# SYNCC-IN/hyperscanning-signal-analysis

Hardware: AMD Instinct MI355X
Metric: MVAR+ffDTF windows/sec, 2x32-ch dyad p=8, 256 freqs (higher is better)
Workload: dtype f64; 1 GPU; C2: 1 dyad(s)/GPU, 2x32 ch @500 Hz, 10 min, 2 s windows 50% overlap (599 windows per dyad), MVAR p=8, 256 freqs 0.5-128 Hz; dyads_per_gpu=1, k1=hop blocks summed once, shared by the overlapping windows (hop 500), k2=block Levinson-Whittle recursion, one workgroup per window, one launch, normalisation=inside K3 (rows of window w by workgroups of window w+lag), parallelism=dyad-sharded x1, gather=none

## Files before the change

hyperscanning_signal_analysis_amd/_lib.py:

```python
from __future__ import annotations

import ctypes
import os
from ctypes import POINTER, c_char_p, c_double, c_int, c_int32, c_int64, c_void_p

_HERE = os.path.dirname(os.path.abspath(__file__))
LIB_PATH = os.path.join(_HERE, "libhypermvar.so")

SIGNATURES = {
    "hmv_version": (c_int, []),
    "hmv_last_error": (c_char_p, []),
    "hmv_pad": (c_int, [c_int]),
    "hmv_set_tuning": (c_int, [c_int, c_int64]),
    "hmv_get_tuning": (c_int64, [c_int]),
    "hmv_yw_workspace_doubles": (c_int64, [c_int, c_int]),
    "hmv_lagcov_f64": (c_int, [c_void_p, c_int64, c_int64, c_void_p, c_void_p, c_int64, c_int, c_int, c_int,
                               c_void_p, c_void_p]),
    "hmv_lagcov_regular_workspace_doubles": (c_int64, [c_int64, c_int, c_int, c_int64, c_int]),
    "hmv_lagcov_regular_f64": (c_int, [c_void_p, c_int64, c_int64, c_int64, c_int64, c_int64, c_int, c_int, c_int,
                                       c_void_p, c_void_p, c_void_p]),
    "hmv_yw_solve_f64": (c_int, [c_void_p, c_int64, c_int, c_int, c_void_p, c_void_p, c_void_p, c_void_p,
                                 c_void_p, c_int64, c_void_p]),
    "hmv_twiddles_f64": (c_int, [c_void_p, c_int, c_double, c_int, c_void_p, c_void_p]),
    "hmv_tf_workspace_doubles": (c_int64, [c_int64, c_int, c_int]),
# ... 95 lines not shown
    "hmv_residuals_workspace_bytes": (c_int64, [c_int64, c_int, c_int]),
    "hmv_residuals_f64": (c_int, [c_void_p, c_int64, c_int64, c_void_p, c_void_p, c_int64, c_int, c_int, c_int, c_void_p,
                                  c_void_p, c_int64, c_void_p, c_int64, c_void_p]),
    "hmv_whiteness_f64": (c_int, [c_void_p, c_int64, c_int, c_int, c_int, c_double] + [c_void_p] * 6),
    "hmv_model_validation_workspace_bytes": (c_int64, [c_int64, c_int, c_int, c_int, c_int]),
    "hmv_model_validation_f64": (c_int, [c_void_p, c_int64, c_int64, c_void_p, c_void_p, c_int64, c_int, c_int, c_int,
                                         c_void_p, c_int, c_double] + [c_void_p] * 7 + [c_int64, c_void_p, c_int64, c_int64,
                                                                                       c_void_p]),
}

FLAG_UNFUSED_NORM = 1
FLAG_YW_TILED = 2
FLAG_YW_ONE_LAUNCH = 4
FLAG_DIRECT_LAGCOV = 8
MEASURE_FFDTF = 0
MEASURE_DDTF = 1
MEASURE_GPDC = 2
CRITERIA = {"AIC": 0, "HQ": 1, "SC": 2}
TUNE_NORM_LAG = 1
TUNE_LAG_GROUP = 2
TUNE_K3_FORM = 3
TUNE_YW_FORM = 4
TUNE_K3_LDS_PAD = 5


_lib = None


class HypermvarLibraryError(ImportError):
    pass


def load():
    global _lib
    if _lib is not None:
        return _lib
    global LIB_PATH
    LIB_PATH = os.environ.get("HYPERMVAR_LIB", LIB_PATH)
    if not os.path.exists(LIB_PATH):
        raise HypermvarLibraryError(
            f"{LIB_PATH} not found: build the HIP library first "
            f"(python -c 'import __graft_entry__ as g; g.build()' or make -C {_HERE}/csrc). "
            "There is no CPU fallback for the MVAR/ffDTF path.")
    lib = ctypes.CDLL(LIB_PATH)
    for name, (res, args) in SIGNATURES.items():
        try:
# ... 17 lines not shown
```

hyperscanning_signal_analysis_amd/csrc/capi.hip:

```cpp
#include "../../include/hypermvar.h"
#include "hmv_kernels.h"

#include <atomic>
#include <cmath>
#include <cstdio>
#include <cstdlib>
#include <cstring>

namespace {
thread_local char g_err[256] = "";

int fail(int code, const char* msg) {
  snprintf(g_err, sizeof(g_err), "%s", msg);
  return code;
}
int pad_of(int m) { return (m < 1 || m > HMV_MAX_CHANNELS) ? -1 : ((m + 15) / 16) * 16; }
inline hipStream_t S(void* s) { return reinterpret_cast<hipStream_t>(s); }
inline size_t align256(size_t b) { return (b + 255) & ~size_t(255); }

constexpr int N_TUNE = 6;
struct TuneRange { long long lo, hi; };
constexpr TuneRange kTuneRange[N_TUNE] = {{0, 0}, {0, 1 << 20}, {0, 3}, {0, 2}, {0, 4}, {0, 140000}};
long long env_knob(const char* name, int key) {
  const char* e = getenv(name);
  if (!e || !*e) return 0;
  char* end = nullptr;
  const long long v = strtoll(e, &end, 10);
  if (end == e || *end != 0 || v < kTuneRange[key].lo || v > kTuneRange[key].hi) {
    fprintf(stderr, "hypermvar: ignoring %s=%s (not an integer in %lld..%lld)\n", name, e, kTuneRange[key].lo,
            kTuneRange[key].hi);
    return 0;
  }
  return v;
}
std::atomic<long long> g_tune[N_TUNE] = {{0}, {env_knob("HYPERMVAR_NORM_LAG", 1)}, {env_knob("HYPERMVAR_LAG_GROUP", 2)},
                                         {env_knob("HYPERMVAR_K3_FORM", 3)}, {env_knob("HYPERMVAR_YW_FORM", 4)},
                                         {env_knob("HYPERMVAR_K3_LDS_PAD", 5)}};
}

namespace hmv {
long long tuning(int key) { return (key >= 1 && key < N_TUNE) ? g_tune[key].load(std::memory_order_relaxed) : -1; }
}

#ifdef HMV_STAMP
static unsigned long long* g_tf_stamps = nullptr;
extern "C" void hmv_debug_set_tf_stamps(void* p) { g_tf_stamps = static_cast<unsigned long long*>(p); }
#endif

extern "C" {

int hmv_version(void) { return HMV_VERSION; }
const char* hmv_last_error(void) { return g_err; }
int hmv_pad(int m) { return pad_of(m); }

int hmv_set_tuning(int key, int64_t value) {
  if (key < 1 || key >= N_TUNE) return fail(-1, "hmv_set_tuning: unknown key");
  if (value < kTuneRange[key].lo || value > kTuneRange[key].hi) return fail(-1, "hmv_set_tuning: value out of range");
  g_tune[key].store(value, std::memory_order_relaxed);
  return 0;
}
// ... 403 lines not shown
    o += align256(sizeof(double) * (size_t)(n < lag ? n : lag) * F * t);
  }
  w.total = o;
  return w;
}
int64_t norm_lag_items(int mp, int F) {
  const int64_t slots = (mp == 64 || mp == 48) ? 1024 : (mp == 32 ? 2048 : 5120);
  int64_t lag = (6 * slots + F - 1) / (F < 1 ? 1 : F);
  if (const int64_t t = hmv::tuning(HMV_TUNE_NORM_LAG)) lag = t;
  return lag < 8 ? 8 : lag;
}
}

int64_t hmv_tf_ffdtf_workspace_bytes(int64_t n_items, int m, int p, int F) {
  const int mp = pad_of(m);
  if (mp < 0 || n_items < 0 || p < 1 || F < 1) return -1;
  return (int64_t)tf_ff_layout(n_items, mp, p, F).total;
}

namespace {
int tf_ffdtf_impl(const char* who, const double* ar, int64_t n_items, int m, int p, const double* tw, int F, double* ffdtf,
                  double* band_out, const int32_t* bin_lo, const int32_t* bin_hi, int n_bands, double* den, double* H,
                  int32_t* info, double pivot_tau, void* workspace, int64_t workspace_bytes, int64_t flags,
                  void* ev_k3_start, void* ev_k3_stop, void* stream, const double* yw_ws = nullptr) {
  auto failw = [&](int code, const char* msg) {
    char buf[200];
    snprintf(buf, sizeof(buf), "%s: %s", who, msg);
    return fail(code, buf);
  };
  const int mp = pad_of(m);
  const bool bands = (band_out != nullptr);
  if (mp < 0) return failw(-1, "channel count must be in 1..64");
  if (p < 1) return failw(-2, "model order must be >= 1");
  if (n_items == 0) return 0;
  if (!ar || !tw || (!ffdtf && !bands) || !den || !info || !workspace || n_items < 0 || F < 1)
    return failw(-4, "null pointer / empty grid");
  if (!(pivot_tau > 0.0) || pivot_tau > 1.0) return failw(-6, "pivot_tau must be in (0, 1]");
  if (bands) {
    if (!bin_lo || !bin_hi || n_bands < 1) return failw(-4, "band bins missing");
    if (F % 32 != 0 || F > hmv::tf_band_max_F(mp) || (flags & HMV_FLAG_UNFUSED_NORM))
      return failw(-10, "in-kernel band sums need F % 32 == 0, F within the row worker's LDS block and the fused normalisation");
  }
  const TfFfWs w = tf_ff_layout(n_items, mp, p, F, bands);
  if ((int64_t)w.total > workspace_bytes) return failw(-7, "workspace too small");
  char* base = static_cast<char*>(workspace);
  const size_t t = (size_t)mp * mp;
  hmv::TfArgs a{};
  a.ar = ar; a.arx = reinterpret_cast<double*>(base + w.off_arx); a.tw = tw;
  a.P = reinterpret_cast<double*>(base + w.off_P); a.rowsum = reinterpret_cast<double*>(base + w.off_rowsum);
  a.H = H;
  a.info = info; a.n_items = n_items; a.F = F; a.p = p; a.m = m; a.tau = pivot_tau;
  const bool fused = bands || (!(flags & HMV_FLAG_UNFUSED_NORM) && (F % 16 == 0) && (reinterpret_cast<uintptr_t>(ffdtf) % 16 == 0));
  const int64_t lag = norm_lag_items(mp, F);
  const int64_t n_fused = fused ? n_items : 0;
  if (n_fused > 0) {
    a.ff = bands ? nullptr : ffdtf; a.den = den; a.fuse_items = n_fused; a.lag = (int)lag;
    if (bands) {
      a.bands = band_out; a.band_lo = reinterpret_cast<const int*>(bin_lo); a.band_hi = reinterpret_cast<const int*>(bin_hi);
      a.nb = n_bands;
    }
    a.wcount = reinterpret_cast<int*>(base + w.off_cnt);
    a.ready = a.wcount + n_items;
    a.missed = a.ready + n_items;
  }
#ifdef HMV_STAMP
  a.stamps = g_tf_stamps;
#endif
  hipStream_t st = S(stream);
  int rc = hmv::launch_tf_inv(a, mp, st, reinterpret_cast<hipEvent_t>(ev_k3_start), reinterpret_cast<hipEvent_t>(ev_k3_stop),
                              yw_ws);
  if (rc) return rc;
  if (n_fused < n_items) {
    const int64_t n_tail = n_items - n_fused;
    double* tail = bands ? reinterpret_cast<double*>(base + w.off_tail) : ffdtf + (size_t)n_fused * m * m * F;
    rc = hmv_ffdtf_norm_f64(a.P + (size_t)n_fused * F * t, a.rowsum + (size_t)n_fused * F * mp, den + (size_t)n_fused * mp,
                            tail, n_tail, F, m, 1, stream);
    if (!rc && bands)
      rc = hmv::launch_band_sums(tail, reinterpret_cast<const int*>(bin_lo), reinterpret_cast<const int*>(bin_hi),
                                 band_out + (size_t)n_fused * m * m * n_bands, n_tail * (long long)m * m, F, n_bands, st);
  }
  return rc;
}
}

int64_t hmv_tf_ffdtf_bands_workspace_bytes(int64_t n_items, int m, int p, int F) {
  const int mp = pad_of(m);
  if (mp < 0 || n_items < 0 || p < 1 || F < 1) return -1;
  return (int64_t)tf_ff_layout(n_items, mp, p, F, true).total;
}

int hmv_tf_ffdtf_f64(const double* ar, int64_t n_items, int m, int p, const double* tw, int F, double* ffdtf,
                     double* den, double* H, int32_t* info, double pivot_tau, void* workspace, int64_t workspace_bytes,
                     int64_t flags, void* ev_k3_start, void* ev_k3_stop, void* stream) {
// ... 42 lines not shown
}
int64_t sliding_bytes(int64_t chunk, int m, int p, int F, int n_bands = 0, bool spectra = false, int measure = MEAS_FFDTF,
                      int64_t q_tiles = -1) {
  const int mp = pad_of(m);
  if (mp < 0 || chunk < 1 || p < 1 || p > HMV_MAX_ORDER || F < 1 || n_bands < 0 || measure < MEAS_FFDTF ||
      measure > MEAS_GPDC)
    return -1;
  return (int64_t)sliding_layout(chunk, mp, p, F, n_bands > 0, spectra, measure, q_tiles).total;
}
struct ForkJoin {
  hipEvent_t fork = nullptr, join = nullptr;
};
ForkJoin* fork_join_events() {
  constexpr int MAXDEV = 64;
  thread_local ForkJoin tl[MAXDEV];
  int dev = 0;
  if (hipGetDevice(&dev) != hipSuccess || dev < 0 || dev >= MAXDEV) return nullptr;
  ForkJoin& e = tl[dev];
  if (!e.fork) {
    if (hipEventCreateWithFlags(&e.fork, hipEventDisableTiming) != hipSuccess) return nullptr;
    if (hipEventCreateWithFlags(&e.join, hipEventDisableTiming) != hipSuccess) return nullptr;
  }
  return &e;
}
}

int64_t hmv_sliding_workspace_bytes(int64_t chunk, int m, int p, int F) { return sliding_bytes(chunk, m, p, F); }

namespace {
struct EnsDesc {
  const int64_t* trial_rec;
  const int64_t* trial_start;
  const int64_t* group_ptr;
  int64_t n_groups, T;
  const int64_t* trial_rec_b = nullptr;
  const int64_t* trial_start_b = nullptr;
  int split = 0;
  const double* R_base = nullptr;
  const int64_t* item_base = nullptr;
};
struct PairDesc {
  const int64_t* rec_b;
  int split;
  const double* R_base;
  const int64_t* base_a;
  const int64_t* base_b;
// ... 70 lines not shown
  if (bands && (!a.bin_lo || !a.bin_hi || a.n_bands < 1)) return fail(-4, "hmv_sliding_ffdtf_f64: band bins missing");
  bool ens_shared = false;
  if (a.ens) {
    if (!a.ens->trial_rec || !a.ens->trial_start || !a.ens->group_ptr)
      return fail(-4, "hmv_sliding_ffdtf_f64: null pointer / empty grid");
    if (a.ens->n_groups < 1) return fail(-10, "hmv_sliding_ffdtf_f64: n_groups must be >= 1");
    if (a.grid_hop != 0 && !ens_grid_ok(a.n_items, a.ens->n_groups, a.n, a.ld, a.ens->T, a.grid_hop, a.grid_nwin))
      return fail(-9, "hmv_sliding_ffdtf_f64: inconsistent regular window grid");
    ens_shared = !a.ens->split && ens_shared_form(a.n, a.p, a.grid_hop, a.flags);
  }
  const SlidingWs w = sliding_layout(a.chunk, mp, a.p, a.F, bands, a.S_out != nullptr, a.measure,
                                     a.ens ? (ens_shared ? ens_q_tiles(a.chunk, a.n, a.p, a.grid_hop, a.grid_nwin) : 0)
                                           : ((a.pairs || a.mix) ? 0 : -1));
  if ((int64_t)w.total > a.workspace_bytes) return fail(-7, "hmv_sliding_ffdtf_f64: workspace too small");
  bool regular = !a.ens && !a.pairs && !a.mix && a.grid_hop > 0 && !(a.flags & HMV_FLAG_DIRECT_LAGCOV);
  if (regular) {
    if (a.grid_nwin < 1 || a.grid_first < 0 || a.n_items % a.grid_nwin != 0 ||
        a.grid_first + (a.grid_nwin - 1) * a.grid_hop + a.n > a.grid_T || a.ld < a.grid_T)
      return fail(-9, "hmv_sliding_ffdtf_f64: inconsistent regular window grid");
    regular = (a.n % a.grid_hop == 0) && (a.n / a.grid_hop >= 2) && (a.n / a.grid_hop <= HMV_MAX_HOPS_PER_WINDOW) &&
              a.grid_hop > a.p;
  }
  hipStream_t st0 = S(a.stream), st1 = S(a.aux_stream);
  const bool split = (a.aux_stream && a.aux_stream != a.stream) && !(a.flags & HMV_FLAG_YW_ONE_LAUNCH);
  ForkJoin* fj = nullptr;
  if (split) {
    fj = fork_join_events();
    if (!fj) return fail(-8, "hmv_sliding_ffdtf_f64: cannot create fork/join events");
  }
  int rc = 0;
  const size_t t = (size_t)mp * mp;
  const int64_t n_chunks = (a.n_items + a.chunk - 1) / a.chunk;
  char* base = static_cast<char*>(a.workspace);
  double* R = reinterpret_cast<double*>(base + w.off_R);
  double* Qb = reinterpret_cast<double*>(base + w.off_Q);
  double* ws = reinterpret_cast<double*>(base + w.off_ws);
  double* ar = reinterpret_cast<double*>(base + w.off_ar);
  double* V = reinterpret_cast<double*>(base + w.off_V);
  void* tfws = base + w.off_tf;
  double* den = reinterpret_cast<double*>(base + w.off_den);
  double* tw = reinterpret_cast<double*>(base + w.off_tw);
  const bool k3_bands = bands && a.measure == MEAS_FFDTF;
  const int64_t tfws_bytes = (int64_t)tf_ff_layout(a.chunk, mp, a.p, a.F, k3_bands).total;
  rc = hmv_twiddles_f64(a.freqs, a.F, a.fs, a.p, tw, st0);
  const size_t ws_item = (size_t)hmv_yw_workspace_doubles(a.m, a.p);
  for (int64_t ci = 0; ci < n_chunks && rc == 0; ++ci) {
    const int64_t i0 = ci * a.chunk;
    const int64_t c = (a.n_items - i0 < a.chunk) ? (a.n_items - i0) : a.chunk;
    double* ar_c = a.ar_out ? a.ar_out + (size_t)i0 * t * a.p : ar;
    double* V_c = a.V_out ? a.V_out + (size_t)i0 * t : V;
    if (a.ens) {
      hmv::LagcovEnsArgs ea{};
      ea.x = a.x; ea.rec_stride = a.rec_stride; ea.ld = a.ld; ea.T = a.ens->T;
      ea.trial_rec = reinterpret_cast<const long long*>(a.ens->trial_rec);
      ea.trial_start = reinterpret_cast<const long long*>(a.ens->trial_start);
      ea.group_ptr = reinterpret_cast<const long long*>(a.ens->group_ptr);
      ea.item_group = reinterpret_cast<const long long*>(a.item_rec + i0);
      ea.item_offset = reinterpret_cast<const long long*>(a.item_start + i0);
      ea.n_items = c; ea.m = a.m; ea.n = a.n; ea.p = a.p; ea.R = R;
      if (ens_shared) {
        ea.it0 = i0; ea.nwin = a.grid_nwin; ea.hop = a.grid_hop; ea.k = (int)(a.n / a.grid_hop); ea.Q = Qb;
      }
      if (a.ens->split) {
        ea.trial_rec_b = reinterpret_cast<const long long*>(a.ens->trial_rec_b);
        ea.trial_start_b = reinterpret_cast<const long long*>(a.ens->trial_start_b);
        ea.split = a.ens->split; ea.R_base = a.ens->R_base;
        ea.item_base = a.ens->item_base ? reinterpret_cast<const long long*>(a.ens->item_base + i0) : nullptr;
        rc = hmv::launch_lagcov_ensemble_split(ea, mp, st0);
// ... 39 lines not shown
      if (rc) break;
    }
    const bool ldl = (a.flags & (HMV_FLAG_YW_TILED | HMV_FLAG_YW_ONE_LAUNCH)) || hmv::tuning(HMV_TUNE_YW_FORM) == 1;
    const bool tiled = (a.flags & HMV_FLAG_YW_TILED) || (ldl && !(a.flags & HMV_FLAG_YW_ONE_LAUNCH) && mp == 64 && c >= 128);
    const int64_t yw_flags = (a.flags & ~(int64_t)(HMV_FLAG_YW_TILED | HMV_FLAG_YW_ONE_LAUNCH)) |
                             (ldl ? (tiled ? HMV_FLAG_YW_TILED : HMV_FLAG_YW_ONE_LAUNCH) : 0);
    const int64_t c0 = (split && tiled && c >= 16) ? (c + 1) / 2 : c, c1 = c - c0;
    if (c1 > 0 && !automatic) {
      int hrc = (int)hipEventRecord(fj->fork, st0);
      if (!hrc) hrc = (int)hipStreamWaitEvent(st1, fj->fork, 0);
      if (hrc) { rc = hrc; break; }
      rc = hmv_yw_solve_f64(R + (size_t)c0 * (a.p + 1) * t, c1, a.m, a.p, ws + (size_t)c0 * ws_item,
                            ar_c + (size_t)c0 * t * a.p, V_c + (size_t)c0 * t, nullptr, a.info_yw + i0 + c0, yw_flags, st1);
      hrc = (int)hipEventRecord(fj->join, st1);
      if (!hrc) hrc = (int)hipStreamWaitEvent(st0, fj->join, 0);
      if (hrc) {
        (void)hipStreamSynchronize(st1);
        if (!rc) rc = hrc;
      }
      if (rc) break;
    }
    const int64_t yw_form = hmv::tuning(HMV_TUNE_YW_FORM);
    const bool from_tiles = !automatic && !a.ar_out && !ldl && (yw_form == 0 || yw_form == 2) && a.measure == MEAS_FFDTF;
    if (!automatic && from_tiles) {
      hmv::YwArgs ya{};
      ya.R = R; ya.n_items = c0; ya.m = a.m; ya.p = a.p; ya.ws = ws; ya.ar = ar_c; ya.V = V_c; ya.info = a.info_yw + i0;
      ya.tiled = -1; ya.no_emit = 1;
      rc = hmv::launch_yw(ya, mp, st0);
    } else if (!automatic) {
      rc = hmv_yw_solve_f64(R, c0, a.m, a.p, ws, ar_c, V_c, nullptr, a.info_yw + i0, yw_flags, st0);
    }
    if (rc) break;
    const bool last = (ci == n_chunks - 1);
    double* Hc = a.S_out ? reinterpret_cast<double*>(base + w.off_H) : nullptr;
    double* full_c = (a.measure == MEAS_FFDTF) ? nullptr
                     : bands ? reinterpret_cast<double*>(base + w.off_full) : a.ffdtf + (size_t)i0 * a.m * a.m * a.F;
    if (a.measure == MEAS_GPDC) {
      rc = hmv::launch_gpdc_sliding(ar_c, V_c, tw, full_c, c, a.F, a.m, mp, a.p, st0);
    } else {
      rc = tf_ffdtf_impl(a.who, ar_c, c, a.m, a.p, tw, a.F,
                         k3_bands ? nullptr : (full_c ? full_c : a.ffdtf + (size_t)i0 * a.m * a.m * a.F),
                         k3_bands ? a.band_out + (size_t)i0 * a.m * a.m * a.n_bands : nullptr, a.bin_lo, a.bin_hi,
                         a.n_bands, den, Hc, a.info_tf + (size_t)i0 * a.F, a.pivot_tau, tfws, tfws_bytes, a.flags,
                         last ? a.ev_k3_start : nullptr, last ? a.ev_k3_stop : nullptr, st0, from_tiles ? ws : nullptr);
    }
    if (!rc && a.measure == MEAS_DDTF) {
      hmv::DdtfArgs da{};
      da.ar = ar_c; da.V = V_c; da.info_yw = a.info_yw + i0;
      da.B = reinterpret_cast<double*>(base + w.off_B); da.G = reinterpret_cast<double*>(base + w.off_G);
      da.freqs = a.freqs; da.fs = a.fs; da.ff = full_c; da.out = full_c;
      da.n_items = c; da.F = a.F; da.m = a.m; da.p = a.p;
      rc = hmv::launch_ddtf_sliding(da, mp, st0);
    }
    if (!rc && a.measure != MEAS_FFDTF && bands)
      rc = hmv::launch_band_sums(full_c, reinterpret_cast<const int*>(a.bin_lo), reinterpret_cast<const int*>(a.bin_hi),
                                 a.band_out + (size_t)i0 * a.m * a.m * a.n_bands, c * (long long)a.m * a.m, a.F,
                                 a.n_bands, st0);
    if (!rc && a.S_out) {
      hmv::SpecArgs sa;
      sa.H = Hc; sa.V = V_c; sa.S = nullptr; sa.S_mmf = a.S_out + (size_t)i0 * a.m * a.m * a.F * 2;
      sa.n_items = c; sa.F = a.F; sa.m = a.m; sa.sym = 1;
      rc = hmv::launch_spectra(sa, mp, st0);
    }
  }
  return rc;
}
}

int64_t hmv_sliding_bands_workspace_bytes(int64_t chunk, int m, int p, int F) { return sliding_bytes(chunk, m, p, F, 1); }

int hmv_sliding_ffdtf_f64(const double* x, int64_t rec_stride, int64_t ld, const int64_t* item_rec,
                          const int64_t* item_start, int64_t n_items, int m, int n, int p,
                          const double* freqs, int F, double fs, double* ffdtf, double* ar_out, double* V_out,
                          int32_t* info_yw, int32_t* info_tf, void* workspace, int64_t workspace_bytes,
                          int64_t chunk, double pivot_tau, int64_t flags, int64_t grid_hop, int64_t grid_first,
                          int64_t grid_nwin, int64_t grid_T, void* ev_k3_start, void* ev_k3_stop, void* stream,
                          void* aux_stream) {
  SlidingArgs a{"hmv_sliding_ffdtf_f64"};
  a.x = x; a.rec_stride = rec_stride; a.ld = ld; a.item_rec = item_rec; a.item_start = item_start; a.n_items = n_items;
  a.m = m; a.n = n; a.p = p; a.freqs = freqs; a.F = F; a.fs = fs;
  a.ffdtf = ffdtf;
  a.ar_out = ar_out; a.V_out = V_out; a.info_yw = info_yw; a.info_tf = info_tf;
  a.workspace = workspace; a.workspace_bytes = workspace_bytes; a.chunk = chunk; a.pivot_tau = pivot_tau; a.flags = flags;
  a.grid_hop = grid_hop; a.grid_first = grid_first; a.grid_nwin = grid_nwin; a.grid_T = grid_T;
  a.ev_k3_start = ev_k3_start; a.ev_k3_stop = ev_k3_stop;
  a.stream = stream; a.aux_stream = aux_stream;
  return sliding_impl(a);
// ... 509 lines not shown
```

hyperscanning_signal_analysis_amd/csrc/hmv_kernels.h:

```cpp
#pragma once
#include <hip/hip_runtime.h>
#include <stdint.h>

namespace hmv {

long long tuning(int key);

struct LagcovArgs {
  const double* x;
  long long rec_stride;
  long long ld;
  const long long* item_rec;
  const long long* item_start;
  long long n_items;
  int m, n, p;
  double* R;
  int blocks;
  long long blk_first, blk_T;
};
int launch_lagcov(const LagcovArgs& a, int m_pad, hipStream_t st);
struct LagcombArgs {
  const double* Q;
  const double* x;
  long long ld, first, hop, T;
// ... 55 lines not shown
struct YwArgs {
  const double* R;
  long long n_items;
  int m, p;
  double* ws;
  double* ar;
  double* V;
  double* Vq_logdet;
  int* info;
  int tiled;
  int only_guarded;
  const int* order;
  int no_emit;
};
struct YwAutoArgs {
  int n;
  double crit_c;
  int* order_out;
  double* crit_out;
};
long long yw_ws_tiles(int p);
int launch_yw(const YwArgs& a, int m_pad, hipStream_t st);
int launch_yw_lwr(const YwArgs& a, int m_pad, hipStream_t st);
int launch_yw_lwr2(const YwArgs& a, int m_pad, hipStream_t st);
int launch_yw_auto(const YwArgs& a, const YwAutoArgs& s, int m_pad, hipStream_t st);
int launch_yw_guarded(const YwArgs& a, int m_pad, hipStream_t st);

struct TfArgs {
  const double* ar;
  const double* arx;
  const double* tw;
  const double* Zin;
  double* detph;
  double* P;
  double* rowsum;
  double* H;
  double* A;
  int* info;
  long long n_items;
  int F, p, m;
  double tau;
  double* ff;
  double* den;
  int* wcount;
  int* ready;
  int* missed;
  long long fuse_items;
  int lag;
  double* bands;
  const int* band_lo;
  const int* band_hi;
  int nb;
  unsigned long long* stamps;
};
int launch_twiddles(const double* freqs, int F, double fs, int p, double* tw, hipStream_t st);
int launch_tf_inv(const TfArgs& a, int m_pad, hipStream_t st, hipEvent_t ev_start = nullptr, hipEvent_t ev_stop = nullptr,
                  const double* yw_ws = nullptr);
int launch_cinv(const TfArgs& a, int m_pad, hipStream_t st);
long long tf_workspace_doubles(long long n_items, int m_pad, int p);
int tf_band_max_F(int m_pad);

struct NormArgs {
  const double* P;
  const double* rowsum;
  double* den;
  double* out;
  long long n_items;
  int F, m, m_pad;
  int normalise;
};
int launch_ffdtf_norm(const NormArgs& a, hipStream_t st);

int launch_trial_mean(const double* in, double* out, long long n, int trials, hipStream_t st);
int launch_ddtf(const double* ff, const double* kappa, double* out, long long n, hipStream_t st);
int launch_band_sums(const double* in, const int* lo, const int* hi, double* out, long long rows, int F, int nb,
                     hipStream_t st);

int launch_transpose_c128(const double* in, double* out, long long n_items, int F, int m, int m_pad, hipStream_t st);

struct SpecArgs {
// ... 117 lines not shown
```

hyperscanning_signal_analysis_amd/csrc/tf_inv.hip:

```cpp
#include "hmv_common.h"
#include "hmv_kernels.h"

namespace hmv {

#ifndef HMV_K3_WGS
#define HMV_K3_WGS 4
#endif

#ifndef HMV_ROW_LOADS_SC1
#define HMV_ROW_LOADS_SC1 0
#endif

#define HMV_LDS_FENCE()                                     \
  do {                                                      \
    __builtin_amdgcn_fence(__ATOMIC_RELEASE, "wavefront");  \
    __builtin_amdgcn_wave_barrier();                        \
    __builtin_amdgcn_fence(__ATOMIC_ACQUIRE, "wavefront");  \
  } while (0)

#ifdef HMV_STAMP
#define HMV_T(idx)                                                                     \
  do {                                                                                 \
    __builtin_amdgcn_sched_barrier(0);                                                 \
    unsigned long long t_;                                                             \
// ... 375 lines not shown
    }
  }
#ifdef HMV_STAMP
  HMV_T(7);
  if (a.stamps && lo == 0) {
    for (int k = 0; k < 8; ++k) a.stamps[(gw * NT + wv) * 8 + k] = tsum[k];
  }
#endif
}

template <int NT, bool GEN>
__global__ void __launch_bounds__(64 * NT, (NT == 4) ? HMV_K3_WGS : 2) tf_inv_kernel(TfArgs a) {
  constexpr int MP = 16 * NT, NG = NT, NSTEP = MP / 4;
  using L = TfLds<NT>;
  constexpr int NR = L::NRING;
  __shared__ double2 smem[L::TOTAL];
  __shared__ int s_orig[MP];
  __shared__ __attribute__((aligned(16))) int s_swp[NR][4];
  __shared__ int s_info;
  __shared__ double s_det[2];

  const int l = lane_id();
  const int wv = uni(threadIdx.x >> 6);
  const int w = (wv + (int)((blockIdx.x * 2654435761u) >> 20)) % NT;
  const int item = uni((int)(blockIdx.x / (unsigned)a.F));
  const int f = uni((int)(blockIdx.x - (unsigned)item * (unsigned)a.F));
  const long long gw = (long long)item * a.F + f;
  const int p = a.p;
  const int i = l >> 4, b = (l >> 2) & 3, j = l & 3;
  const int rowl = 4 * b + i;
  const int colw = 4 * w + j;

  double2* Pbuf = smem;
  double2* Nbuf = Pbuf + L::PBUF;
  double2* Srow = Nbuf + NR * L::NBUF;
  double2* swapb = Srow + L::SROW + wv * 32;
  double* rsum = reinterpret_cast<double*>(Srow + L::SROW + L::SWAPB);

  double re[NG][4], im[NG][4];
  [[maybe_unused]] double zscale = 1.0;
#ifdef HMV_STAMP
  unsigned long long tsum[8] = {0, 0, 0, 0, 0, 0, 0, 0}, tlast;
  asm volatile("s_memtime %0\n\ts_waitcnt lgkmcnt(0)" : "=s"(tlast)::"memory");
#endif

  if constexpr (GEN) {
    const double2* Zi = reinterpret_cast<const double2*>(a.Zin) + (size_t)gw * MP * MP + (size_t)rowl * MP + colw;
#pragma unroll
    for (int Ig = 0; Ig < NG; ++Ig)
// ... 366 lines not shown
  );
}

#ifndef HMV_K3A_INC
#define HMV_K3A_INC "tf_inv64_body.inc"
#endif
#include HMV_K3A_INC
#ifndef HMV_K3A_WGS
#ifdef HMV_STAMP
#define HMV_K3A_WGS 4
#else
#define HMV_K3A_WGS 5
#endif
#endif
static_assert(K3A_PBUF == 0 && K3A_NBUF == 16 * TfLds<4>::PBUF && K3A_RSUM == 16 * (TfLds<4>::TOTAL - TfLds<4>::RSUM),
              "LDS map of the generated body and of the epilogue disagree");

__global__ void __launch_bounds__(256, HMV_K3A_WGS) tf_inv64_asm_kernel(TfArgs a) {
  constexpr int NT = 4;
  __shared__ __attribute__((aligned(16))) unsigned char lds[K3A_LDS_TOTAL];
  int* s_orig = reinterpret_cast<int*>(lds + K3A_SORIG);
  int* s_flag = reinterpret_cast<int*>(lds + K3A_SINFO);
  const int wv = uni(threadIdx.x >> 6);
  const int w = (wv + (int)((blockIdx.x * 2654435761u) >> 20)) % NT;
  const int item = uni((int)(blockIdx.x / (unsigned)a.F));
  const int f = uni((int)(blockIdx.x - (unsigned)item * (unsigned)a.F));
  const long long gw = (long long)item * a.F + f;
  if (w == 0) {
    const int l = lane_id();
    s_orig[l] = l;
    if (l == 0) *s_flag = 0;
  }
  const int p = a.p, P2 = (p + 1) >> 1;
  const double* arx = a.arx + ((size_t)item * NT + w) * (size_t)(16 * 64 * 2) * P2;
  const double* tw = a.tw + (size_t)f * p * 2;
  const double tau = a.tau;
  const unsigned ldsbase = (unsigned)(uintptr_t)lds;
  double acc[32];
#ifdef HMV_STAMP
  unsigned long long tsum[8] = {0, 0, 0, 0, 0, 0, 0, 0}, tlast = 0, q0, q1, q2, q3;
  unsigned tl32;
  K3A_BODY_STAMPED(acc, arx, tw, p, w, tau, ldsbase, q0, q1, q2, q3, tl32);
  {
    const unsigned long long d[8] = {q0 & 0xffffffffull, q0 >> 32, q1 & 0xffffffffull, q1 >> 32,
                                     q2 & 0xffffffffull, q2 >> 32, q3 & 0xffffffffull, q3 >> 32};
    tsum[0] = d[0]; tsum[2] = d[1]; tsum[3] = d[2] + d[3] + d[4]; tsum[1] = d[5] + d[6] + d[7];
    unsigned long long now;
    asm volatile("s_memtime %0\n\ts_waitcnt lgkmcnt(0)" : "=s"(now)::"memory");
    tlast = (now & ~0xffffffffull) | tl32;
// ... 65 lines not shown
}

int launch_twiddles(const double* freqs, int F, double fs, int p, double* tw, hipStream_t st) {
  const int n = F * p;
  hipLaunchKernelGGL(twiddle_kernel, dim3((n + 255) / 256), dim3(256), 0, st, freqs, F, fs, p, tw);
  return (int)hipGetLastError();
}

int tf_band_max_F(int m_pad) {
  switch (m_pad) {
    case 16: return (2 * TfLds<1>::TOTAL) & ~31;
    case 32: return (2 * TfLds<2>::TOTAL) & ~31;
    case 48: return (2 * TfLds<3>::TOTAL) & ~31;
    case 64: return (2 * TfLds<4>::TOTAL) & ~31;
  }
  return 0;
}

long long tf_workspace_doubles(long long n_items, int m_pad, int p) {
  return n_items * (long long)m_pad * m_pad * 2 * ((p + 1) / 2);
}

int launch_tf_inv(const TfArgs& a_in, int m_pad, hipStream_t st, hipEvent_t ev_start, hipEvent_t ev_stop,
                  const double* yw_ws) {
  TfArgs a = a_in;
  if (a.n_items == 0 || a.F == 0) return 0;
  const bool fused = ((a.ff != nullptr || a.bands != nullptr) && a.fuse_items > 0);
  if (fused) {
    if (!a.P || !a.den || !a.wcount || !a.ready || !a.missed || a.lag < 1) return -3;
    if (a.bands && (!a.band_lo || !a.band_hi || a.nb < 1 || a.F % 32 != 0 || a.F > tf_band_max_F(m_pad) || a.A)) return -3;
    if (const hipError_t e = hipMemsetAsync(a.wcount, 0, sizeof(int) * (2 * (size_t)a.n_items + 1), st)) return (int)e;
  } else {
    a.ff = nullptr;
    a.bands = nullptr;
  }
  const long long n = a.n_items * (long long)a.F;
  const dim3 grid((unsigned)n);
  const long long slots = a.n_items * (long long)m_pad * m_pad * ((a.p + 1) / 2);
  const dim3 pgrid((unsigned)((slots + 255) / 256));
  double* arx = const_cast<double*>(a.arx);
  const long long ws_item = yw_ws_tiles(a.p) * (long long)m_pad * m_pad;
#define HMV_AR_PACK(NT)                                                                                                  \
  if (yw_ws) hipLaunchKernelGGL((ar_pack_kernel<NT, true>), pgrid, dim3(256), 0, st, a.ar, yw_ws, ws_item, arx, a.n_items, a.p); \
  else hipLaunchKernelGGL((ar_pack_kernel<NT, false>), pgrid, dim3(256), 0, st, a.ar, yw_ws, ws_item, arx, a.n_items, a.p)
  switch (m_pad) {
    case 16: HMV_AR_PACK(1); break;
    case 32: HMV_AR_PACK(2); break;
    case 48: HMV_AR_PACK(3); break;
    case 64: HMV_AR_PACK(4); break;
    default: return -1;
  }
#undef HMV_AR_PACK
  if (ev_start)
    if (const hipError_t e = hipEventRecord(ev_start, st)) return (int)e;
  switch (m_pad) {
    case 16: hipLaunchKernelGGL((tf_inv_kernel<1, false>), grid, dim3(64), 0, st, a); break;
    case 32: hipLaunchKernelGGL((tf_inv_kernel<2, false>), grid, dim3(128), 0, st, a); break;
    case 48: hipLaunchKernelGGL((tf_inv_kernel<3, false>), grid, dim3(192), 0, st, a); break;
    case 64:
      if (tuning(5) > 0) {
        (void)hipFuncSetAttribute(reinterpret_cast<const void*>(&tf_inv64_asm_kernel), hipFuncAttributeMaxDynamicSharedMemorySize,
                                  (int)tuning(5));
        (void)hipFuncSetAttribute(reinterpret_cast<const void*>(&tf_inv_kernel<4, false>),
                                  hipFuncAttributeMaxDynamicSharedMemorySize, (int)tuning(5));
      }
      if ((tuning(3 ) != 1 || a.bands != nullptr) && a.A == nullptr)
        hipLaunchKernelGGL(tf_inv64_asm_kernel, grid, dim3(256), (unsigned)tuning(5 ), st, a);
      else
        hipLaunchKernelGGL((tf_inv_kernel<4, false>), grid, dim3(256), (unsigned)tuning(5), st, a);
      break;
  }
  if (ev_stop)
    if (const hipError_t e = hipEventRecord(ev_stop, st)) return (int)e;
  if (fused) {
    const long long tail_rows = (a.fuse_items > a.lag ? a.lag : a.fuse_items) * a.m;
    const dim3 mgrid((unsigned)(tail_rows > 2048 ? 2048 : (tail_rows < 256 ? 256 : tail_rows)));
    switch (m_pad) {
      case 16: hipLaunchKernelGGL(norm_missed_kernel<1>, mgrid, dim3(64), 0, st, a); break;
      case 32: hipLaunchKernelGGL(norm_missed_kernel<2>, mgrid, dim3(128), 0, st, a); break;
      case 48: hipLaunchKernelGGL(norm_missed_kernel<3>, mgrid, dim3(192), 0, st, a); break;
      case 64: hipLaunchKernelGGL(norm_missed_kernel<4>, mgrid, dim3(256), 0, st, a); break;
    }
  }
  return (int)hipGetLastError();
}

int launch_cinv(const TfArgs& a_in, int m_pad, hipStream_t st) {
  TfArgs a = a_in;
  a.ff = nullptr;
  a.bands = nullptr;
  a.fuse_items = 0;
  const long long n = a.n_items * (long long)a.F;
  if (n == 0) return 0;
  const dim3 grid((unsigned)n);
// ... 12 lines not shown
```

hyperscanning_signal_analysis_amd/csrc/yw_lwr.hip:

```cpp
#include "yw_lwr_core.h"

namespace hmv {

template <int NT, bool VQ, bool LEGACY = false>
__global__ void __launch_bounds__(256, 3) yw_lwr_kernel(YwArgs a) {
  yw_lwr_body<NT, VQ, false, LEGACY>(a, YwAutoArgs{});
}

static int launch_yw_lwr_legacy(const YwArgs& a, int m_pad, hipStream_t st) {
  const dim3 grid((unsigned)a.n_items), block(256);
  const bool vq = (a.Vq_logdet != nullptr);
  switch (m_pad) {
    case 16: if (vq) hipLaunchKernelGGL((yw_lwr_kernel<1, true, true>), grid, block, 0, st, a);
             else hipLaunchKernelGGL((yw_lwr_kernel<1, false, true>), grid, block, 0, st, a); break;
    case 32: if (vq) hipLaunchKernelGGL((yw_lwr_kernel<2, true, true>), grid, block, 0, st, a);
             else hipLaunchKernelGGL((yw_lwr_kernel<2, false, true>), grid, block, 0, st, a); break;
    case 48: if (vq) hipLaunchKernelGGL((yw_lwr_kernel<3, true, true>), grid, block, 0, st, a);
             else hipLaunchKernelGGL((yw_lwr_kernel<3, false, true>), grid, block, 0, st, a); break;
    case 64: if (vq) hipLaunchKernelGGL((yw_lwr_kernel<4, true, true>), grid, block, 0, st, a);
             else hipLaunchKernelGGL((yw_lwr_kernel<4, false, true>), grid, block, 0, st, a); break;
    default: return -1;
  }
  return (int)hipGetLastError();
}

int launch_yw_lwr(const YwArgs& a, int m_pad, hipStream_t st) {
  if (a.n_items == 0) return 0;
  if (tuning(4 ) == 3) return launch_yw_lwr2(a, m_pad, st);
  if (tuning(4) == 4) return launch_yw_lwr_legacy(a, m_pad, st);
  const dim3 grid((unsigned)a.n_items), block(256);
  const bool vq = (a.Vq_logdet != nullptr);
  switch (m_pad) {
    case 16: if (vq) hipLaunchKernelGGL((yw_lwr_kernel<1, true>), grid, block, 0, st, a);
             else hipLaunchKernelGGL((yw_lwr_kernel<1, false>), grid, block, 0, st, a); break;
    case 32: if (vq) hipLaunchKernelGGL((yw_lwr_kernel<2, true>), grid, block, 0, st, a);
             else hipLaunchKernelGGL((yw_lwr_kernel<2, false>), grid, block, 0, st, a); break;
    case 48: if (vq) hipLaunchKernelGGL((yw_lwr_kernel<3, true>), grid, block, 0, st, a);
             else hipLaunchKernelGGL((yw_lwr_kernel<3, false>), grid, block, 0, st, a); break;
    case 64: if (vq) hipLaunchKernelGGL((yw_lwr_kernel<4, true>), grid, block, 0, st, a);
             else hipLaunchKernelGGL((yw_lwr_kernel<4, false>), grid, block, 0, st, a); break;
    default: return -1;
  }
  return (int)hipGetLastError();
}

}
```

include/hypermvar.h:

```cpp
#ifndef HYPERMVAR_H
#define HYPERMVAR_H

#include <stdint.h>

#ifdef __cplusplus
extern "C" {
#endif

#define HMV_VERSION 160
#define HMV_MAX_CHANNELS 64
#define HMV_MAX_ORDER 32

int hmv_version(void);
const char* hmv_last_error(void);
int hmv_pad(int m);
#define HMV_TUNE_NORM_LAG 1
#define HMV_TUNE_LAG_GROUP 2
#define HMV_TUNE_K3_FORM 3
#define HMV_TUNE_YW_FORM 4
#define HMV_TUNE_K3_LDS_PAD 5
int hmv_set_tuning(int key, int64_t value);
int64_t hmv_get_tuning(int key);
int64_t hmv_yw_workspace_doubles(int m, int p);

int hmv_lagcov_f64(const double* x, int64_t rec_stride, int64_t ld,
                   const int64_t* item_rec, const int64_t* item_start, int64_t n_items,
                   int m, int n, int p, double* R, void* stream);

#define HMV_MAX_HOPS_PER_WINDOW 8
int64_t hmv_lagcov_regular_workspace_doubles(int64_t n_win, int m, int n, int64_t hop, int p);
int hmv_lagcov_regular_f64(const double* x, int64_t ld, int64_t T, int64_t first, int64_t hop, int64_t n_win,
                           int m, int n, int p, double* R, double* workspace, void* stream);

int hmv_yw_solve_f64(const double* R, int64_t n_items, int m, int p, double* ws,
                     double* ar, double* V, double* vq_logdet, int32_t* info, int64_t flags, void* stream);

int hmv_twiddles_f64(const double* freqs, int F, double fs, int p, double* tw, void* stream);

int64_t hmv_tf_workspace_doubles(int64_t n_items, int m, int p);
int hmv_tf_f64(const double* ar, int64_t n_items, int m, int p, const double* tw, int F,
               double* P, double* rowsum, double* H, double* A, int32_t* info,
               double pivot_tau, double* ws, void* stream);

// ... 217 lines not shown
```

Measured before the change: 59280 windows/s.

## Split YW solve tail wave onto aux stream to overlap with K3 transfer-function kernel

The block Levinson solve is split at a whole-wave boundary chosen from CU count and kernel occupancy. The partial last wave runs on the auxiliary stream, while the transfer-function/ffDTF kernel (K3) starts on the first items in the main stream. K3 and its AR packing are launched in two segments via a new item0 offset, and the second segment waits on a join event. This aims to hide the underfilled tail wave of the YW kernel. In exchange it adds an extra launch, event synchronisation and a new tuning knob, and the fused lagged normalisation must still be correct across the segment boundary.

```diff
diff --git a/hyperscanning_signal_analysis_amd/_lib.py b/hyperscanning_signal_analysis_amd/_lib.py
--- a/hyperscanning_signal_analysis_amd/_lib.py
+++ b/hyperscanning_signal_analysis_amd/_lib.py
@@ -141,6 +141,7 @@
 TUNE_K3_FORM = 3
 TUNE_YW_FORM = 4
 TUNE_K3_LDS_PAD = 5
+TUNE_K3_SPLIT = 6
 
 
 _lib = None
diff --git a/hyperscanning_signal_analysis_amd/csrc/capi.hip b/hyperscanning_signal_analysis_amd/csrc/capi.hip
--- a/hyperscanning_signal_analysis_amd/csrc/capi.hip
+++ b/hyperscanning_signal_analysis_amd/csrc/capi.hip
@@ -18,9 +18,9 @@
 inline hipStream_t S(void* s) { return reinterpret_cast<hipStream_t>(s); }
 inline size_t align256(size_t b) { return (b + 255) & ~size_t(255); }
 
-constexpr int N_TUNE = 6;
+constexpr int N_TUNE = 7;
 struct TuneRange { long long lo, hi; };
-constexpr TuneRange kTuneRange[N_TUNE] = {{0, 0}, {0, 1 << 20}, {0, 3}, {0, 2}, {0, 4}, {0, 140000}};
+constexpr TuneRange kTuneRange[N_TUNE] = {{0, 0}, {0, 1 << 20}, {0, 3}, {0, 2}, {0, 4}, {0, 140000}, {-1, 1 << 20}};
 long long env_knob(const char* name, int key) {
   const char* e = getenv(name);
   if (!e || !*e) return 0;
@@ -35,7 +35,7 @@
 }
 std::atomic<long long> g_tune[N_TUNE] = {{0}, {env_knob("HYPERMVAR_NORM_LAG", 1)}, {env_knob("HYPERMVAR_LAG_GROUP", 2)},
                                          {env_knob("HYPERMVAR_K3_FORM", 3)}, {env_knob("HYPERMVAR_YW_FORM", 4)},
-                                         {env_knob("HYPERMVAR_K3_LDS_PAD", 5)}};
+                                         {env_knob("HYPERMVAR_K3_LDS_PAD", 5)}, {env_knob("HYPERMVAR_K3_SPLIT", 6)}};
 }
 
 namespace hmv {
@@ -485,7 +485,8 @@
 int tf_ffdtf_impl(const char* who, const double* ar, int64_t n_items, int m, int p, const double* tw, int F, double* ffdtf,
                   double* band_out, const int32_t* bin_lo, const int32_t* bin_hi, int n_bands, double* den, double* H,
                   int32_t* info, double pivot_tau, void* workspace, int64_t workspace_bytes, int64_t flags,
-                  void* ev_k3_start, void* ev_k3_stop, void* stream, const double* yw_ws = nullptr) {
+                  void* ev_k3_start, void* ev_k3_stop, void* stream, const double* yw_ws = nullptr,
+                  hmv::TfSplit* k3_split = nullptr) {
   auto failw = [&](int code, const char* msg) {
     char buf[200];
     snprintf(buf, sizeof(buf), "%s: %s", who, msg);
@@ -531,7 +532,7 @@
 #endif
   hipStream_t st = S(stream);
   int rc = hmv::launch_tf_inv(a, mp, st, reinterpret_cast<hipEvent_t>(ev_k3_start), reinterpret_cast<hipEvent_t>(ev_k3_stop),
-                              yw_ws);
+                              yw_ws, k3_split);
   if (rc) return rc;
   if (n_fused < n_items) {
     const int64_t n_tail = n_items - n_fused;
@@ -620,6 +621,30 @@
     if (hipEventCreateWithFlags(&e.join, hipEventDisableTiming) != hipSuccess) return nullptr;
   }
   return &e;
+}
+int64_t k3_split_point(int64_t c, int mp, int64_t lag) {
+  const int64_t t = hmv::tuning(HMV_TUNE_K3_SPLIT);
+  int64_t c0 = t;
+  if (t < 0) return 0;
+  if (t == 0) {
+    constexpr int MAXDEV = 64;
+    struct Shape { int cus = 0, occ[4] = {0, 0, 0, 0}; };
+    thread_local Shape tl[MAXDEV];
+    int dev = 0;
+    if (hipGetDevice(&dev) != hipSuccess || dev < 0 || dev >= MAXDEV || mp < 16 || mp > 64) return 0;
+    Shape& d = tl[dev];
+    int& occ = d.occ[mp / 16 - 1];
+    if (d.cus == 0 && hipDeviceGetAttribute(&d.cus, hipDeviceAttributeMultiprocessorCount, dev) != hipSuccess) d.cus = -1;
+    if (occ == 0 && (occ = hmv::yw_lwr_occupancy(mp)) == 0) occ = -1;
+    if (d.cus < 1 || occ < 1) {
+      (void)hipGetLastError();
+      return 0;
+    }
+    const int64_t k = c / d.cus, r = c % d.cus;
+    if (k < 1 || k >= occ || r == 0) return 0;
+    c0 = c - r;
+  }
+  return (c0 >= lag && c0 < c) ? c0 : 0;
 }
 }
 
@@ -736,9 +761,12 @@
               a.grid_hop > a.p;
   }
   hipStream_t st0 = S(a.stream), st1 = S(a.aux_stream);
-  const bool split = (a.aux_stream && a.aux_stream != a.stream) && !(a.flags & HMV_FLAG_YW_ONE_LAUNCH);
+  const bool two = (a.aux_stream && a.aux_stream != a.stream);
+  const bool split = two && !(a.flags & HMV_FLAG_YW_ONE_LAUNCH);
+  const bool k3_split = two && !automatic && a.measure == MEAS_FFDTF && !a.S_out && !a.ar_out && !a.V_out &&
+                        !(a.flags & (HMV_FLAG_YW_TILED | HMV_FLAG_YW_ONE_LAUNCH));
   ForkJoin* fj = nullptr;
-  if (split) {
+  if (split || k3_split) {
     fj = fork_join_events();
     if (!fj) return fail(-8, "hmv_sliding_ffdtf_f64: cannot create fork/join events");
   }
@@ -758,6 +786,12 @@
   const int64_t tfws_bytes = (int64_t)tf_ff_layout(a.chunk, mp, a.p, a.F, k3_bands).total;
   rc = hmv_twiddles_f64(a.freqs, a.F, a.fs, a.p, tw, st0);
   const size_t ws_item = (size_t)hmv_yw_workspace_doubles(a.m, a.p);
+  hmv::TfSplit sp{};
+  auto join_k3_split = [&]() {
+    if (sp.join && !sp.joined)
+      if (hipStreamWaitEvent(st0, sp.join, 0) != hipSuccess) (void)hipStreamSynchronize(st1);
+    sp.joined = true;
+  };
   for (int64_t ci = 0; ci < n_chunks && rc == 0; ++ci) {
     const int64_t i0 = ci * a.chunk;
     const int64_t c = (a.n_items - i0 < a.chunk) ? (a.n_items - i0) : a.chunk;
@@ -843,11 +877,29 @@
     }
     const int64_t yw_form = hmv::tuning(HMV_TUNE_YW_FORM);
     const bool from_tiles = !automatic && !a.ar_out && !ldl && (yw_form == 0 || yw_form == 2) && a.measure == MEAS_FFDTF;
+    sp = hmv::TfSplit{};
     if (!automatic && from_tiles) {
+      const int64_t s0 = k3_split ? k3_split_point(c, mp, norm_lag_items(mp, a.F)) : 0;
       hmv::YwArgs ya{};
-      ya.R = R; ya.n_items = c0; ya.m = a.m; ya.p = a.p; ya.ws = ws; ya.ar = ar_c; ya.V = V_c; ya.info = a.info_yw + i0;
+      ya.R = R; ya.n_items = s0 ? s0 : c0; ya.m = a.m; ya.p = a.p; ya.ws = ws; ya.ar = ar_c; ya.V = V_c; ya.info = a.info_yw + i0;
       ya.tiled = -1; ya.no_emit = 1;
       rc = hmv::launch_yw(ya, mp, st0);
+      if (!rc && s0) {
+        int hrc = (int)hipEventRecord(fj->fork, st0);
+        if (!hrc) hrc = (int)hipStreamWaitEvent(st1, fj->fork, 0);
+        if (hrc) { rc = hrc; break; }
+        hmv::YwArgs yb = ya;
+        yb.R = R + (size_t)s0 * (a.p + 1) * t; yb.n_items = c - s0; yb.ws = ws + (size_t)s0 * ws_item;
+        yb.ar = ar_c + (size_t)s0 * t * a.p; yb.V = V_c + (size_t)s0 * t; yb.info = a.info_yw + i0 + s0;
+        rc = hmv::launch_yw(yb, mp, st1);
+        hrc = (int)hipEventRecord(fj->join, st1);
+        if (hrc) {
+          (void)hipStreamSynchronize(st1);
+          if (!rc) rc = hrc;
+        } else {
+          sp.c0 = s0; sp.join = fj->join;
+        }
+      }
     } else if (!automatic) {
       rc = hmv_yw_solve_f64(R, c0, a.m, a.p, ws, ar_c, V_c, nullptr, a.info_yw + i0, yw_flags, st0);
     }
@@ -863,8 +915,9 @@
                          k3_bands ? nullptr : (full_c ? full_c : a.ffdtf + (size_t)i0 * a.m * a.m * a.F),
                          k3_bands ? a.band_out + (size_t)i0 * a.m * a.m * a.n_bands : nullptr, a.bin_lo, a.bin_hi,
                          a.n_bands, den, Hc, a.info_tf + (size_t)i0 * a.F, a.pivot_tau, tfws, tfws_bytes, a.flags,
-                         last ? a.ev_k3_start : nullptr, last ? a.ev_k3_stop : nullptr, st0, from_tiles ? ws : nullptr);
+                         last ? a.ev_k3_start : nullptr, last ? a.ev_k3_stop : nullptr, st0, from_tiles ? ws : nullptr, &sp);
     }
+    join_k3_split();
     if (!rc && a.measure == MEAS_DDTF) {
       hmv::DdtfArgs da{};
       da.ar = ar_c; da.V = V_c; da.info_yw = a.info_yw + i0;
@@ -884,6 +937,7 @@
       rc = hmv::launch_spectra(sa, mp, st0);
     }
   }
+  join_k3_split();
   return rc;
 }
 }
diff --git a/hyperscanning_signal_analysis_amd/csrc/hmv_kernels.h b/hyperscanning_signal_analysis_amd/csrc/hmv_kernels.h
--- a/hyperscanning_signal_analysis_amd/csrc/hmv_kernels.h
+++ b/hyperscanning_signal_analysis_amd/csrc/hmv_kernels.h
@@ -101,6 +101,7 @@
 long long yw_ws_tiles(int p);
 int launch_yw(const YwArgs& a, int m_pad, hipStream_t st);
 int launch_yw_lwr(const YwArgs& a, int m_pad, hipStream_t st);
+int yw_lwr_occupancy(int m_pad);
 int launch_yw_lwr2(const YwArgs& a, int m_pad, hipStream_t st);
 int launch_yw_auto(const YwArgs& a, const YwAutoArgs& s, int m_pad, hipStream_t st);
 int launch_yw_guarded(const YwArgs& a, int m_pad, hipStream_t st);
@@ -131,10 +132,16 @@
   const int* band_hi;
   int nb;
   unsigned long long* stamps;
+  int item0;
+};
+struct TfSplit {
+  long long c0 = 0;
+  hipEvent_t join = nullptr;
+  bool joined = false;
 };
 int launch_twiddles(const double* freqs, int F, double fs, int p, double* tw, hipStream_t st);
 int launch_tf_inv(const TfArgs& a, int m_pad, hipStream_t st, hipEvent_t ev_start = nullptr, hipEvent_t ev_stop = nullptr,
-                  const double* yw_ws = nullptr);
+                  const double* yw_ws = nullptr, TfSplit* split = nullptr);
 int launch_cinv(const TfArgs& a, int m_pad, hipStream_t st);
 long long tf_workspace_doubles(long long n_items, int m_pad, int p);
 int tf_band_max_F(int m_pad);
diff --git a/hyperscanning_signal_analysis_amd/csrc/tf_inv.hip b/hyperscanning_signal_analysis_amd/csrc/tf_inv.hip
--- a/hyperscanning_signal_analysis_amd/csrc/tf_inv.hip
+++ b/hyperscanning_signal_analysis_amd/csrc/tf_inv.hip
@@ -421,9 +421,10 @@
 
   const int l = lane_id();
   const int wv = uni(threadIdx.x >> 6);
-  const int w = (wv + (int)((blockIdx.x * 2654435761u) >> 20)) % NT;
-  const int item = uni((int)(blockIdx.x / (unsigned)a.F));
-  const int f = uni((int)(blockIdx.x - (unsigned)item * (unsigned)a.F));
+  const unsigned bid = blockIdx.x + (unsigned)a.item0 * (unsigned)a.F;
+  const int w = (wv + (int)((bid * 2654435761u) >> 20)) % NT;
+  const int item = uni((int)(bid / (unsigned)a.F));
+  const int f = uni((int)(bid - (unsigned)item * (unsigned)a.F));
   const long long gw = (long long)item * a.F + f;
   const int p = a.p;
   const int i = l >> 4, b = (l >> 2) & 3, j = l & 3;
@@ -836,9 +837,10 @@
   int* s_orig = reinterpret_cast<int*>(lds + K3A_SORIG);
   int* s_flag = reinterpret_cast<int*>(lds + K3A_SINFO);
   const int wv = uni(threadIdx.x >> 6);
-  const int w = (wv + (int)((blockIdx.x * 2654435761u) >> 20)) % NT;
-  const int item = uni((int)(blockIdx.x / (unsigned)a.F));
-  const int f = uni((int)(blockIdx.x - (unsigned)item * (unsigned)a.F));
+  const unsigned bid = blockIdx.x + (unsigned)a.item0 * (unsigned)a.F;
+  const int w = (wv + (int)((bid * 2654435761u) >> 20)) % NT;
+  const int item = uni((int)(bid / (unsigned)a.F));
+  const int f = uni((int)(bid - (unsigned)item * (unsigned)a.F));
   const long long gw = (long long)item * a.F + f;
   if (w == 0) {
     const int l = lane_id();
@@ -950,9 +952,10 @@
 }
 
 int launch_tf_inv(const TfArgs& a_in, int m_pad, hipStream_t st, hipEvent_t ev_start, hipEvent_t ev_stop,
-                  const double* yw_ws) {
+                  const double* yw_ws, TfSplit* split) {
   TfArgs a = a_in;
   if (a.n_items == 0 || a.F == 0) return 0;
+  if (m_pad != 16 && m_pad != 32 && m_pad != 48 && m_pad != 64) return -1;
   const bool fused = ((a.ff != nullptr || a.bands != nullptr) && a.fuse_items > 0);
   if (fused) {
     if (!a.P || !a.den || !a.wcount || !a.ready || !a.missed || a.lag < 1) return -3;
@@ -962,42 +965,52 @@
     a.ff = nullptr;
     a.bands = nullptr;
   }
-  const long long n = a.n_items * (long long)a.F;
-  const dim3 grid((unsigned)n);
-  const long long slots = a.n_items * (long long)m_pad * m_pad * ((a.p + 1) / 2);
-  const dim3 pgrid((unsigned)((slots + 255) / 256));
-  double* arx = const_cast<double*>(a.arx);
+  const long long c0 = (split && split->join && split->c0 > 0 && split->c0 < a.n_items) ? split->c0 : a.n_items;
+  const long long per_item = (long long)m_pad * m_pad * ((a.p + 1) / 2);
   const long long ws_item = yw_ws_tiles(a.p) * (long long)m_pad * m_pad;
-#define HMV_AR_PACK(NT)                                                                                                  \
-  if (yw_ws) hipLaunchKernelGGL((ar_pack_kernel<NT, true>), pgrid, dim3(256), 0, st, a.ar, yw_ws, ws_item, arx, a.n_items, a.p); \
-  else hipLaunchKernelGGL((ar_pack_kernel<NT, false>), pgrid, dim3(256), 0, st, a.ar, yw_ws, ws_item, arx, a.n_items, a.p)
-  switch (m_pad) {
-    case 16: HMV_AR_PACK(1); break;
-    case 32: HMV_AR_PACK(2); break;
-    case 48: HMV_AR_PACK(3); break;
-    case 64: HMV_AR_PACK(4); break;
-    default: return -1;
-  }
+  for (long long i0 = 0, ni = c0; i0 < a.n_items; i0 += ni, ni = a.n_items - i0) {
+    if (i0 > 0) {
+      if (const hipError_t e = hipStreamWaitEvent(st, split->join, 0)) return (int)e;
+      split->joined = true;
+    }
+    const dim3 pgrid((unsigned)((ni * per_item + 255) / 256));
+    const double* ar = a.ar + (size_t)i0 * m_pad * m_pad * a.p;
+    const double* wsp = yw_ws ? yw_ws + (size_t)i0 * ws_item : nullptr;
+    double* arx = const_cast<double*>(a.arx) + (size_t)i0 * per_item * 2;
+#define HMV_AR_PACK(NT)                                                                                             \
+  if (yw_ws) hipLaunchKernelGGL((ar_pack_kernel<NT, true>), pgrid, dim3(256), 0, st, ar, wsp, ws_item, arx, ni, a.p); \
+  else hipLaunchKernelGGL((ar_pack_kernel<NT, false>), pgrid, dim3(256), 0, st, ar, wsp, ws_item, arx, ni, a.p)
+    switch (m_pad) {
+      case 16: HMV_AR_PACK(1); break;
+      case 32: HMV_AR_PACK(2); break;
+      case 48: HMV_AR_PACK(3); break;
+      case 64: HMV_AR_PACK(4); break;
+    }
 #undef HMV_AR_PACK
-  if (ev_start)
-    if (const hipError_t e = hipEventRecord(ev_start, st)) return (int)e;
-  switch (m_pad) {
-    case 16: hipLaunchKernelGGL((tf_inv_kernel<1, false>), grid, dim3(64), 0, st, a); break;
-    case 32: hipLaunchKernelGGL((tf_inv_kernel<2, false>), grid, dim3(128), 0, st, a); break;
-    case 48: hipLaunchKernelGGL((tf_inv_kernel<3, false>), grid, dim3(192), 0, st, a); break;
-    case 64:
-      if (tuning(5) > 0) {
-        (void)hipFuncSetAttribute(reinterpret_cast<const void*>(&tf_inv64_asm_kernel), hipFuncAttributeMaxDynamicSharedMemorySize,
-                                  (int)tuning(5));
-        (void)hipFuncSetAttribute(reinterpret_cast<const void*>(&tf_inv_kernel<4, false>),
-                                  hipFuncAttributeMaxDynamicSharedMemorySize, (int)tuning(5));
-      }
-      if ((tuning(3 ) != 1 || a.bands != nullptr) && a.A == nullptr)
-        hipLaunchKernelGGL(tf_inv64_asm_kernel, grid, dim3(256), (unsigned)tuning(5 ), st, a);
-      else
-        hipLaunchKernelGGL((tf_inv_kernel<4, false>), grid, dim3(256), (unsigned)tuning(5), st, a);
-      break;
-  }
+    if (ev_start && i0 == 0)
+      if (const hipError_t e = hipEventRecord(ev_start, st)) return (int)e;
+    a.item0 = (int)i0;
+    const dim3 grid((unsigned)(ni * (long long)a.F));
+    switch (m_pad) {
+      case 16: hipLaunchKernelGGL((tf_inv_kernel<1, false>), grid, dim3(64), 0, st, a); break;
+      case 32: hipLaunchKernelGGL((tf_inv_kernel<2, false>), grid, dim3(128), 0, st, a); break;
+      case 48: hipLaunchKernelGGL((tf_inv_kernel<3, false>), grid, dim3(192), 0, st, a); break;
+      case 64:
+        if (tuning(5) > 0) {
+          (void)hipFuncSetAttribute(reinterpret_cast<const void*>(&tf_inv64_asm_kernel),
+                                    hipFuncAttributeMaxDynamicSharedMemorySize, (int)tuning(5));
+          (void)hipFuncSetAttribute(reinterpret_cast<const void*>(&tf_inv_kernel<4, false>),
+                                    hipFuncAttributeMaxDynamicSharedMemorySize, (int)tuning(5));
+        }
+        if ((tuning(3 ) != 1 || a.bands != nullptr) && a.A == nullptr)
+          hipLaunchKernelGGL(tf_inv64_asm_kernel, grid, dim3(256), (unsigned)tuning(5 ), st, a);
+        else
+          hipLaunchKernelGGL((tf_inv_kernel<4, false>), grid, dim3(256), (unsigned)tuning(5), st, a);
+        break;
+    }
+    if (const hipError_t e = hipGetLastError()) return (int)e;
+  }
+  a.item0 = 0;
   if (ev_stop)
     if (const hipError_t e = hipEventRecord(ev_stop, st)) return (int)e;
   if (fused) {
diff --git a/hyperscanning_signal_analysis_amd/csrc/yw_lwr.hip b/hyperscanning_signal_analysis_amd/csrc/yw_lwr.hip
--- a/hyperscanning_signal_analysis_amd/csrc/yw_lwr.hip
+++ b/hyperscanning_signal_analysis_amd/csrc/yw_lwr.hip
@@ -44,4 +44,18 @@
   return (int)hipGetLastError();
 }
 
+int yw_lwr_occupancy(int m_pad) {
+  if (tuning(4 ) == 3 || tuning(4) == 4) return 0;
+  int occ = 0;
+  hipError_t e = hipErrorInvalidValue;
+  switch (m_pad) {
+    case 16: e = hipOccupancyMaxActiveBlocksPerMultiprocessor(&occ, yw_lwr_kernel<1, false>, 256, 0); break;
+    case 32: e = hipOccupancyMaxActiveBlocksPerMultiprocessor(&occ, yw_lwr_kernel<2, false>, 256, 0); break;
+    case 48: e = hipOccupancyMaxActiveBlocksPerMultiprocessor(&occ, yw_lwr_kernel<3, false>, 256, 0); break;
+    case 64: e = hipOccupancyMaxActiveBlocksPerMultiprocessor(&occ, yw_lwr_kernel<4, false>, 256, 0); break;
+    default: return 0;
+  }
+  return (e == hipSuccess && occ > 0) ? occ : 0;
 }
+
+}
diff --git a/include/hypermvar.h b/include/hypermvar.h
--- a/include/hypermvar.h
+++ b/include/hypermvar.h
@@ -19,6 +19,7 @@
 #define HMV_TUNE_K3_FORM 3
 #define HMV_TUNE_YW_FORM 4
 #define HMV_TUNE_K3_LDS_PAD 5
+#define HMV_TUNE_K3_SPLIT 6
 int hmv_set_tuning(int key, int64_t value);
 int64_t hmv_get_tuning(int key);
 int64_t hmv_yw_workspace_doubles(int m, int p);
```

After: 60910 windows/s, median of 6. +2.8%, better.
